# ameli/gaussian-process-param-estimation

Measured on NVIDIA B200. Metric: loglik+grad evals/s (Matern nu=2.5 dense n=20k, FP64), higher is better.
Workload: dtype f64

## Files before the change

gaussian-process-param-estimation_b200/csrc/gp_gemm.cu:

```cuda
#include "gp_common.cuh"
#include "gp_internal.h"
#include <cuda.h>
#include <algorithm>
#include <mutex>
#include <set>
#include <utility>
#include <vector>

namespace gp {

std::atomic<unsigned long long> g_launch_count{0};

struct GemmProfile {
    bool on = false;
    std::vector<cudaEvent_t> pool;
    size_t used = 0;
    double flops = 0.0;
    long long launches = 0;
    cudaEvent_t ref = nullptr;
};
static GemmProfile g_prof;
static std::mutex g_prof_mutex;

static std::mutex g_cfg_mutex;
static std::set<std::pair<int, const void*>> g_cfg_done;

int configure_once(const void* func, int smem_bytes) {
    int dev = 0;
    GP_CUDA_CHECK(cudaGetDevice(&dev));
    std::lock_guard<std::mutex> lock(g_cfg_mutex);
    std::pair<int, const void*> key(dev, func);
    if (g_cfg_done.count(key)) return 0;
    GP_CUDA_CHECK(cudaFuncSetAttribute(func, cudaFuncAttributeMaxDynamicSharedMemorySize, smem_bytes));
    g_cfg_done.insert(key);
    return 0;
}

static cudaEvent_t profile_begin(double flops, cudaStream_t stream) {
    if (!g_prof.on) return nullptr;
    std::lock_guard<std::mutex> lock(g_prof_mutex);
    while (g_prof.pool.size() < g_prof.used + 2) {
        cudaEvent_t e;
        if (cudaEventCreate(&e) != cudaSuccess) return nullptr;
        g_prof.pool.push_back(e);
    }
    cudaEvent_t e0 = g_prof.pool[g_prof.used++];
    cudaEvent_t e1 = g_prof.pool[g_prof.used++];
    g_prof.flops += flops;
    g_prof.launches++;
    cudaEventRecord(e0, stream);
    return e1;
}

static double tile_flops(int tiles_m, int tiles_n, int bn, int K, int krange, int tmask) {
    double kt = 0.0;
    for (int tm = 0; tm < tiles_m; ++tm) {
        int lim = ((tm + 1) * 128) / bn;
        int ncols = (tmask == TM_LOWER) ? (lim < tiles_n ? lim : tiles_n) : tiles_n;
        if (krange == KR_FULL) kt += (double)ncols * K;
        else if (krange == KR_A_LOWER) kt += (double)ncols * ((tm + 1) * 128 < K ? (tm + 1) * 128 : K);
        else for (int tn = 0; tn < ncols; ++tn) {
            int kb = (krange == KR_B_LOWER) ? tn * bn : (tm * 128 > tn * bn ? tm * 128 : tn * bn);
            kt += (double)(K - (kb < K ? kb : K));
        }
    }
    return 2.0 * 128.0 * bn * kt;
}

constexpr int BM = 128, WM = 64, WN = 32, MI = WM / 8, NI = WN / 8;
constexpr int RASTER_GROUP = 8;

template <int BN_>
struct TCfg {
    static constexpr int BN = BN_;
    static constexpr int BK = 16;
    static constexpr int STAGES = (BN_ == 128) ? 6 : 4;
    static constexpr int WARPS_N = BN_ / WN;
    static constexpr int CONSUMER_WARPS = (BM / WM) * WARPS_N;
    static constexpr int THREADS = (CONSUMER_WARPS + 1) * 32;
    static constexpr int A_BYTES = BM * BK * 8, B_BYTES = BN_ * BK * 8, STAGE_BYTES = A_BYTES + B_BYTES;
    static constexpr int SMEM = STAGES * STAGE_BYTES + 2048;
    static constexpr int MIN_CTAS = (BN_ == 128) ? 1 : 2;
};

__device__ __forceinline__ void mbar_init(uint32_t bar, int count) {
    asm volatile("mbarrier.init.shared::cta.b64 [%0], %1;\n" ::"r"(bar), "r"(count));
}
__device__ __forceinline__ void mbar_expect_tx(uint32_t bar, uint32_t bytes) {
    asm volatile("mbarrier.arrive.expect_tx.shared::cta.b64 _, [%0], %1;\n" ::"r"(bar), "r"(bytes) : "memory");
}
__device__ __forceinline__ void mbar_arrive(uint32_t bar) {
    asm volatile("mbarrier.arrive.shared::cta.b64 _, [%0];\n" ::"r"(bar) : "memory");
}
__device__ __forceinline__ void mbar_arrive_after(uint32_t bar, uint32_t value) {
    asm volatile(
        "{\n"
        ".reg .pred q;\n"
        "setp.ne.u32 q, %1, 0x7ff7a5c3;\n"
        "@q mbarrier.arrive.shared::cta.b64 _, [%0];\n"
        "@!q mbarrier.arrive.shared::cta.b64 _, [%0];\n"
        "}\n" ::"r"(bar), "r"(value) : "memory");
}
__device__ __forceinline__ void mbar_wait(uint32_t bar, uint32_t parity) {
    uint32_t done;
    do {
        asm volatile(
            "{\n"
            ".reg .pred p;\n"
            "mbarrier.try_wait.parity.shared::cta.b64 p, [%1], %2;\n"
            "selp.u32 %0, 1, 0, p;\n"
            "}\n" : "=r"(done) : "r"(bar), "r"(parity) : "memory");
    } while (!done);
}
__device__ __forceinline__ void tma_load_2d(uint32_t dst, const CUtensorMap* map, uint32_t bar, int c0, int c1) {
    asm volatile(
        "cp.async.bulk.tensor.2d.shared::cluster.global.mbarrier::complete_tx::bytes [%0], [%1, {%3, %4}], [%2];\n"
        ::"r"(dst), "l"(reinterpret_cast<uint64_t>(map)), "r"(bar), "r"(c0), "r"(c1) : "memory");
}
__device__ __forceinline__ void tma_load_5d(uint32_t dst, const CUtensorMap* map, uint32_t bar, int c0, int c1, int c2,
                                            int c3, int c4) {
    asm volatile(
        "cp.async.bulk.tensor.5d.shared::cluster.global.mbarrier::complete_tx::bytes [%0], [%1, {%3, %4, %5, %6, %7}], [%2];\n"
        ::"r"(dst), "l"(reinterpret_cast<uint64_t>(map)), "r"(bar), "r"(c0), "r"(c1), "r"(c2), "r"(c3), "r"(c4) : "memory");
}

template <int T>
__device__ __forceinline__ uint32_t frag_off(int mn, int kk, int t) {
    if (T == 0) {
        int chunk = (kk | ((t >> 1) << 2)) ^ (mn & 7);
        return (uint32_t)(mn * 128 + (chunk << 4) + ((t & 1) << 3));
    }
    int r = (kk & 1) | ((t & 1) << 1) | ((t >> 1) << 2) | ((kk >> 1) << 3);
    int ml = mn & 15;
    int chunk = (ml >> 1) ^ (r & 7);
    return (uint32_t)((mn >> 4) * 2048 + r * 128 + (chunk << 4) + ((ml & 1) << 3));
}

__device__ __forceinline__ double lds_f64(uint32_t addr) {
    double v;
    asm volatile("ld.shared.f64 %0, [%1];\n" : "=d"(v) : "r"(addr));
    return v;
}

template <int AT, int BT, int BN_>
__global__ void __launch_bounds__(TCfg<BN_>::THREADS, TCfg<BN_>::MIN_CTAS)
dgemm_tma_kernel(const __grid_constant__ CUtensorMap mapA, const __grid_constant__ CUtensorMap mapB, double* C, int64_t ldc,
                 int tiles_m, int tiles_n, int K, double alpha, double beta, int krange, int tmask,
                 const int* __restrict__ kbeg_tab, const int* __restrict__ kend_tab) {
    using G = TCfg<BN_>;
    constexpr int BN = G::BN, BK = G::BK, STAGES = G::STAGES;
    extern __shared__ __align__(16) unsigned char smem_raw[];

    int bid = blockIdx.x;
    int group_sz = RASTER_GROUP * tiles_n;
    int grp = bid / group_sz;
    int first_m = grp * RASTER_GROUP;
    int rows_in_grp = min(RASTER_GROUP, tiles_m - first_m);
    int rem = bid - grp * group_sz;
    int tm = first_m + rem % rows_in_grp;
    int tn = rem / rows_in_grp;
    const int m0 = tm * BM, n0 = tn * BN;
    if (tmask == TM_LOWER && n0 >= m0 + BM) return;

    int kbeg = 0, kend = K;
    if (krange == KR_A_LOWER) kend = min(K, m0 + BM);
    else if (krange == KR_B_LOWER) kbeg = min(n0, K);
    else if (krange == KR_TN_LOWER) kbeg = min(max(m0, n0), K);
    if (kbeg_tab) kbeg = max(kbeg, min(kbeg_tab[tm], K));
    if (kend_tab) kend = min(kend, kend_tab[tm]);
    kbeg = (kbeg / BK) * BK;
    const int KT = max(0, (kend - kbeg) / BK);

    const uint32_t base = ((uint32_t)__cvta_generic_to_shared(smem_raw) + 1023u) & ~1023u;
    const uint32_t bars = base + STAGES * G::STAGE_BYTES;
    const int tid = threadIdx.x, lane = tid & 31, warp = tid >> 5;

    if (tid == 0) {
#pragma unroll
        for (int s = 0; s < STAGES; ++s) {
            mbar_init(bars + 8 * s, 1);
            mbar_init(bars + 8 * (STAGES + s), G::CONSUMER_WARPS);
        }
        asm volatile("fence.mbarrier_init.release.cluster;\n" ::: "memory");
    }
    __syncthreads();

    if (warp == G::CONSUMER_WARPS) {
        if (lane == 0) {
            asm volatile("prefetch.tensormap [%0];\n" ::"l"(reinterpret_cast<uint64_t>(&mapA)) : "memory");
            asm volatile("prefetch.tensormap [%0];\n" ::"l"(reinterpret_cast<uint64_t>(&mapB)) : "memory");
            for (int kt = 0; kt < KT; ++kt) {
                const int s = kt % STAGES;
                if (kt >= STAGES) mbar_wait(bars + 8 * (STAGES + s), ((kt / STAGES) - 1) & 1);
                const uint32_t full = bars + 8 * s;
                const uint32_t sa = base + s * G::STAGE_BYTES, sb = sa + G::A_BYTES;
                const int k0 = kbeg + kt * BK;
                mbar_expect_tx(full, G::STAGE_BYTES);
                if (AT == 0) {
                    tma_load_2d(sa, &mapA, full, k0, m0);
                } else {
#pragma unroll
                    for (int j = 0; j < BM / 16; ++j) tma_load_5d(sa + j * 2048, &mapA, full, m0 + 16 * j, 0, 0, k0 >> 3, 0);
                }
                if (BT == 0) {
                    tma_load_2d(sb, &mapB, full, k0, n0);
                } else {
#pragma unroll
                    for (int j = 0; j < BN / 16; ++j) tma_load_5d(sb + j * 2048, &mapB, full, n0 + 16 * j, 0, 0, k0 >> 3, 0);
                }
            }
        }
        return;
    }

    const int g = lane >> 2, t = lane & 3;
    const int wm = (warp / G::WARPS_N) * WM, wn = (warp % G::WARPS_N) * WN;

    double acc[MI][NI][2];
#pragma unroll
    for (int i = 0; i < MI; ++i)
#pragma unroll
        for (int j = 0; j < NI; ++j) acc[i][j][0] = acc[i][j][1] = 0.0;

    if (beta != 0.0) {
        constexpr int LINES = BM * BN / 16;
        constexpr int CT = G::CONSUMER_WARPS * 32;
#pragma unroll
        for (int i = 0; i < LINES / CT; ++i) {
            int line = tid + i * CT;
            const double* pc = C + (int64_t)(m0 + line / (BN / 16)) * ldc + n0 + ((line % (BN / 16)) << 4);
            asm volatile("prefetch.global.L2 [%0];" ::"l"(pc));
        }
    }

    uint32_t aoff[4], boff[4];
#pragma unroll
    for (int kk = 0; kk < 4; ++kk) {
        aoff[kk] = frag_off<AT>(wm + g, kk, t);
        boff[kk] = frag_off<BT>(wn + g, kk, t);
    }
    for (int kt = 0; kt < KT; ++kt) {
        const int s = kt % STAGES;
        mbar_wait(bars + 8 * s, (kt / STAGES) & 1);
        const uint32_t sa = base + s * G::STAGE_BYTES, sb = sa + G::A_BYTES;
        uint32_t dep = 0;
#pragma unroll
        for (int kk = 0; kk < 4; ++kk) {
            double a[MI], b[NI];
#pragma unroll
            for (int i = 0; i < MI; ++i) {
                uint32_t o = (AT == 0) ? aoff[kk] + i * 1024 : ((aoff[kk] ^ ((i & 1) << 6)) + (i >> 1) * 2048);
                a[i] = lds_f64(sa + o);
            }
#pragma unroll
            for (int j = 0; j < NI; ++j) {
                uint32_t o = (BT == 0) ? boff[kk] + j * 1024 : ((boff[kk] ^ ((j & 1) << 6)) + (j >> 1) * 2048);
                b[j] = lds_f64(sb + o);
            }
#pragma unroll
            for (int i = 0; i < MI; ++i) dep ^= (uint32_t)__double2hiint(a[i]);
#pragma unroll
            for (int j = 0; j < NI; ++j) dep ^= (uint32_t)__double2hiint(b[j]);
#pragma unroll
            for (int i = 0; i < MI; ++i)
#pragma unroll
                for (int j = 0; j < NI; ++j) dmma884(acc[i][j][0], acc[i][j][1], a[i], b[j]);
        }
        dep = __reduce_xor_sync(0xffffffffu, dep);
        if (lane == 0) mbar_arrive_after(bars + 8 * (STAGES + s), dep);
    }

    const bool diag = (tmask == TM_LOWER) && (n0 + BN - 1 > m0);
    if (beta != 0.0 && !diag) {
#pragma unroll
        for (int i = 0; i < MI; i += 2) {
            double2 o[2][NI];
#pragma unroll
            for (int ii = 0; ii < 2; ++ii)
#pragma unroll
                for (int j = 0; j < NI; ++j)
                    o[ii][j] = *reinterpret_cast<const double2*>(C + (int64_t)(m0 + wm + (i + ii) * 8 + g) * ldc + n0 + wn + j * 8 + 2 * t);
#pragma unroll
            for (int ii = 0; ii < 2; ++ii)
#pragma unroll
                for (int j = 0; j < NI; ++j) {
                    double2 v;
                    v.x = alpha * acc[i + ii][j][0] + beta * o[ii][j].x;
                    v.y = alpha * acc[i + ii][j][1] + beta * o[ii][j].y;
                    *reinterpret_cast<double2*>(C + (int64_t)(m0 + wm + (i + ii) * 8 + g) * ldc + n0 + wn + j * 8 + 2 * t) = v;
                }
        }
        return;
    }
#pragma unroll
    for (int i = 0; i < MI; ++i) {
        const int grow = m0 + wm + i * 8 + g;
        double* crow = C + (int64_t)grow * ldc;
#pragma unroll
        for (int j = 0; j < NI; ++j) {
            const int gcol = n0 + wn + j * 8 + 2 * t;
            if (diag && gcol > grow) continue;
            double2 v;
            v.x = alpha * acc[i][j][0];
            v.y = alpha * acc[i][j][1];
            double2* p = reinterpret_cast<double2*>(crow + gcol);
            if (beta != 0.0) {
                double2 o = *p;
                v.x += beta * o.x;
                v.y += beta * o.y;
            }
            if (diag && gcol + 1 > grow) {
                crow[gcol] = v.x;
            } else {
                *p = v;
            }
        }
    }
}

typedef CUresult (*EncodeTiledFn)(CUtensorMap*, CUtensorMapDataType, cuuint32_t, void*, const cuuint64_t*, const cuuint64_t*,
                                  const cuuint32_t*, const cuuint32_t*, CUtensorMapInterleave, CUtensorMapSwizzle,
                                  CUtensorMapL2promotion, CUtensorMapFloatOOBfill);
static EncodeTiledFn g_encode = nullptr;
static int g_encode_state = 0;

static int encode_init() {
    if (g_encode_state) return g_encode_state;
    void* fn = nullptr;
    cudaDriverEntryPointQueryResult q;
    if (cudaGetDriverEntryPoint("cuTensorMapEncodeTiled", &fn, cudaEnableDefault, &q) != cudaSuccess || !fn ||
        q != cudaDriverEntryPointSuccess) {
        (void)cudaGetLastError();
        g_encode_state = -1;
        return -1;
    }
    g_encode = (EncodeTiledFn)fn;
    g_encode_state = 1;
    return 1;
}

static int make_map(CUtensorMap* map, int T, const double* P, int64_t ld, int mn, int K, int rows_per_box) {
    cuuint32_t es[5] = {1, 1, 1, 1, 1};
    CUresult r;
    if (T == 0) {
        cuuint64_t dims[2] = {(cuuint64_t)K, (cuuint64_t)mn};
        cuuint64_t strides[1] = {(cuuint64_t)ld * 8};
        cuuint32_t box[2] = {16, (cuuint32_t)rows_per_box};
        r = g_encode(map, CU_TENSOR_MAP_DATA_TYPE_FLOAT64, 2, (void*)P, dims, strides, box, es, CU_TENSOR_MAP_INTERLEAVE_NONE,
                     CU_TENSOR_MAP_SWIZZLE_128B, CU_TENSOR_MAP_L2_PROMOTION_L2_128B, CU_TENSOR_MAP_FLOAT_OOB_FILL_NONE);
    } else {
        cuuint64_t dims[5] = {(cuuint64_t)mn, 2, 2, (cuuint64_t)(K / 8), 2};
        cuuint64_t strides[4] = {(cuuint64_t)ld * 16, (cuuint64_t)ld * 8, (cuuint64_t)ld * 64, (cuuint64_t)ld * 32};
        cuuint32_t box[5] = {16, 2, 2, 2, 2};
        r = g_encode(map, CU_TENSOR_MAP_DATA_TYPE_FLOAT64, 5, (void*)P, dims, strides, box, es, CU_TENSOR_MAP_INTERLEAVE_NONE,
                     CU_TENSOR_MAP_SWIZZLE_128B, CU_TENSOR_MAP_L2_PROMOTION_L2_128B, CU_TENSOR_MAP_FLOAT_OOB_FILL_NONE);
    }
    return r == CUDA_SUCCESS ? 0 : -(int)r - 2000;
}

template <int AT, int BT, int BN_>
static int launch_tma_inst(double* C, int64_t ldc, const double* A, int64_t lda, const double* B, int64_t ldb,
                           int M, int N, int K, double alpha, double beta, int krange, int tmask, cudaStream_t stream,
                           const int* kbeg_tab, const int* kend_tab) {
    using G = TCfg<BN_>;
    if (K % G::BK) return -1;
    int tiles_m = M / BM, tiles_n = N / BN_;
    if (tiles_m == 0 || tiles_n == 0) return 0;
    int rc = configure_once((const void*)dgemm_tma_kernel<AT, BT, BN_>, G::SMEM);
    if (rc) return rc;
    const int Kmap = K > 0 ? K : 32;
    CUtensorMap mapA, mapB;
    if ((rc = make_map(&mapA, AT, A, lda, M, Kmap, BM))) return rc;
    if ((rc = make_map(&mapB, BT, B, ldb, N, Kmap, BN_))) return rc;
    cudaEvent_t e1 = profile_begin(tile_flops(tiles_m, tiles_n, BN_, K, krange, tmask), stream);
    dgemm_tma_kernel<AT, BT, BN_><<<tiles_m * tiles_n, G::THREADS, G::SMEM, stream>>>(
        mapA, mapB, C, ldc, tiles_m, tiles_n, K, alpha, beta, krange, tmask, kbeg_tab, kend_tab);
    if (e1) cudaEventRecord(e1, stream);
    GP_COUNT(1);
    GP_LAUNCH_CHECK();
    return 0;
}

static int launch_tma_bn64(int at, int bt, double* C, int64_t ldc, const double* A, int64_t lda, const double* B, int64_t ldb,
                           int M, int N, int K, double alpha, double beta, int krange, int tmask, cudaStream_t stream,
                           const int* kbeg_tab, const int* kend_tab) {
    if (at == 0 && bt == 0) return launch_tma_inst<0, 0, 64>(C, ldc, A, lda, B, ldb, M, N, K, alpha, beta, krange, tmask, stream, kbeg_tab, kend_tab);
    if (at == 0 && bt == 1) return launch_tma_inst<0, 1, 64>(C, ldc, A, lda, B, ldb, M, N, K, alpha, beta, krange, tmask, stream, kbeg_tab, kend_tab);
    if (at == 1 && bt == 1) return launch_tma_inst<1, 1, 64>(C, ldc, A, lda, B, ldb, M, N, K, alpha, beta, krange, tmask, stream, kbeg_tab, kend_tab);
    if (at == 1 && bt == 0) return launch_tma_inst<1, 0, 64>(C, ldc, A, lda, B, ldb, M, N, K, alpha, beta, krange, tmask, stream, kbeg_tab, kend_tab);
    return -4;
}

static int check_args(int at, int bt, const double* C, int64_t ldc, const double* A, int64_t lda, const double* B,
                      int64_t ldb, int M, int N, int K, bool ktab) {
    if (M < 0 || N < 0 || K < 0 || (M % BM) || (N % 128) || (K % 32)) return -1;
    if ((lda & 1) || (ldb & 1) || (ldc & 1)) return -2;
    if (((uintptr_t)A | (uintptr_t)B | (uintptr_t)C) & 15) return -3;
    const bool in_place = !ktab && C == A && C != B && ldc == lda && at == 0 && bt == 0 && N == 128;
    if ((C == A || C == B) && !in_place) return -6;
    if (encode_init() != 1) return -7;
    return in_place ? 128 : 64;
}

int launch_dgemm(int at, int bt, double* C, int64_t ldc, const double* A, int64_t lda, const double* B, int64_t ldb,
                 int M, int N, int K, double alpha, double beta, int krange, int tmask, cudaStream_t stream) {
    const int bn = check_args(at, bt, C, ldc, A, lda, B, ldb, M, N, K, false);
    if (bn < 0) return bn;
    if (bn == 128)
        return launch_tma_inst<0, 0, 128>(C, ldc, A, lda, B, ldb, M, N, K, alpha, beta, krange, tmask, stream, nullptr, nullptr);
    return launch_tma_bn64(at, bt, C, ldc, A, lda, B, ldb, M, N, K, alpha, beta, krange, tmask, stream, nullptr, nullptr);
}

int launch_dgemm_ktab(int at, int bt, double* C, int64_t ldc, const double* A, int64_t lda, const double* B, int64_t ldb,
                      int M, int N, int K, double alpha, double beta, const int* kbeg_tab, const int* kend_tab,
                      cudaStream_t stream) {
    const int bn = check_args(at, bt, C, ldc, A, lda, B, ldb, M, N, K, true);
    if (bn < 0) return bn;
    return launch_tma_bn64(at, bt, C, ldc, A, lda, B, ldb, M, N, K, alpha, beta, KR_FULL, TM_ALL, stream, kbeg_tab, kend_tab);
}


int profile_enable(int on) {
    g_prof.on = on != 0;
    g_prof.used = 0;
    g_prof.flops = 0.0;
    g_prof.launches = 0;
    if (g_prof.on) {
        if (!g_prof.ref) GP_CUDA_CHECK(cudaEventCreate(&g_prof.ref));
        GP_CUDA_CHECK(cudaDeviceSynchronize());
        GP_CUDA_CHECK(cudaEventRecord(g_prof.ref, 0));
        GP_CUDA_CHECK(cudaDeviceSynchronize());
    }
    return 0;
}

int profile_read(double* ms_sum, double* ms_union, double* flops, long long* launches) {
    GP_CUDA_CHECK(cudaDeviceSynchronize());
    std::vector<std::pair<float, float>> iv;
    double total = 0.0;
    for (size_t i = 0; i + 1 < g_prof.used; i += 2) {
        float t0 = 0.f, t1 = 0.f;
        GP_CUDA_CHECK(cudaEventElapsedTime(&t0, g_prof.ref, g_prof.pool[i]));
        GP_CUDA_CHECK(cudaEventElapsedTime(&t1, g_prof.ref, g_prof.pool[i + 1]));
        total += (double)t1 - (double)t0;
        iv.push_back(std::make_pair(t0, t1));
    }
    std::sort(iv.begin(), iv.end());
    double uni = 0.0;
    float cur0 = 0.f, cur1 = -1.f;
    for (size_t i = 0; i < iv.size(); ++i) {
        if (cur1 < cur0 || iv[i].first > cur1) {
            if (cur1 >= cur0) uni += (double)cur1 - (double)cur0;
            cur0 = iv[i].first;
            cur1 = iv[i].second;
        } else if (iv[i].second > cur1) {
            cur1 = iv[i].second;
        }
    }
    if (cur1 >= cur0) uni += (double)cur1 - (double)cur0;
    *ms_sum = total;
    *ms_union = uni;
    *flops = g_prof.flops;
    *launches = g_prof.launches;
    return 0;
}

}
```

gaussian-process-param-estimation_b200/csrc/gp_loglik.cu:

```cuda
#include "../../include/gpgp.h"
#include "gp_common.cuh"
#include "gp_internal.h"
#include "gp_matern.cuh"

namespace gp {

constexpr int MAXP = 16;
constexpr int LMAXD = 8;

__global__ void __launch_bounds__(256)
gram_partial_kernel(const double* __restrict__ A, const double* __restrict__ B, int nrows, int p, int64_t ld,
                    double* partial) {
    __shared__ double sa[64 * MAXP], sb[64 * MAXP];
    const int tid = threadIdx.x;
    const int a = tid / p, b = tid - a * p;
    double acc = 0.0;
    int rows_per_cta = (nrows + gridDim.x - 1) / gridDim.x;
    int r0 = blockIdx.x * rows_per_cta, r1 = min(nrows, r0 + rows_per_cta);
    for (int base = r0; base < r1; base += 64) {
        int cnt = min(64, r1 - base);
        __syncthreads();
        for (int idx = tid; idx < cnt * p; idx += 256) {
            int r = idx / p, c = idx - r * p;
            sa[idx] = A[(int64_t)(base + r) * ld + c];
            sb[idx] = B[(int64_t)(base + r) * ld + c];
        }
        __syncthreads();
        if (tid < p * p)
            for (int r = 0; r < cnt; ++r) acc += sa[r * p + a] * sb[r * p + b];
    }
    if (tid < p * p) partial[(int64_t)blockIdx.x * p * p + tid] = acc;
}

__global__ void sum_partials_kernel(const double* partial, int nparts, int width, double* out) {
    int t = blockIdx.x * blockDim.x + threadIdx.x;
    if (t >= width) return;
    double s = 0.0;
    for (int i = 0; i < nparts; ++i) s += partial[(int64_t)i * width + t];
    out[t] = s;
}

template <int MODE, bool WITH_DK>
__global__ void __launch_bounds__(256)
trace_tiles_kernel(const double* __restrict__ Ainv, int n, int npad, const double* __restrict__ pts, int d,
                   MaternParams mp, double* partial) {
    __shared__ double pr[LMAXD][128], pc[LMAXD][128];
    __shared__ double red[32];
    int b = blockIdx.x;
    int tm = (int)((sqrt(8.0 * b + 1.0) - 1.0) * 0.5);
    while ((tm + 1) * (tm + 2) / 2 <= b) ++tm;
    while (tm * (tm + 1) / 2 > b) --tm;
    int tn = b - tm * (tm + 1) / 2;
    const int m0 = tm * 128, n0 = tn * 128, tid = threadIdx.x;
    if (WITH_DK) {
        for (int idx = tid; idx < 128 * d; idx += 256) {
            int r = idx / d, k = idx - r * d;
            pr[k][r] = (m0 + r < n) ? pts[(int64_t)(m0 + r) * d + k] : 0.0;
            pc[k][r] = (n0 + r < n) ? pts[(int64_t)(n0 + r) * d + k] : 0.0;
        }
        __syncthreads();
    }
    double t1 = 0.0, t2 = 0.0, t3 = 0.0;
    const int tx = tid & 63, ty = tid >> 6;
    for (int r = ty; r < 128; r += 4) {
        int gi = m0 + r;
        if (gi >= n) break;
        double2 v = *reinterpret_cast<const double2*>(Ainv + (int64_t)gi * npad + n0 + 2 * tx);
        double vals[2] = {v.x, v.y};
#pragma unroll
        for (int e = 0; e < 2; ++e) {
            int gj = n0 + 2 * tx + e;
            if (gj > gi || gj >= n) continue;
            double a = vals[e];
            if (gj == gi) {
                t1 += a;
                t2 += a * a;
            } else {
                t2 += 2.0 * a * a;
                if (WITH_DK) {
                    double s = 0.0, ud = 0.0;
#pragma unroll
                    for (int k = 0; k < LMAXD; ++k)
                        if (k < d) {
                            double t = (pr[k][r] - pc[k][2 * tx + e]) * mp.inv_scale[k];
                            s += t * t;
                            if (k == mp.ddim) ud = t * t;
                        }
                    double val, dval;
                    matern_value_drho<MODE>(sqrt(s), mp, &val, &dval);
                    if (mp.ddim >= 0) dval = (s > 0.0) ? dval * (ud / s) * mp.inv_scale[mp.ddim] : 0.0;
                    t3 += 2.0 * a * dval;
                }
            }
        }
    }
    t1 = block_sum(t1, red);
    t2 = block_sum(t2, red);
    t3 = block_sum(t3, red);
    if (tid == 0) {
        partial[(int64_t)b * 3 + 0] = t1;
        partial[(int64_t)b * 3 + 1] = t2;
        partial[(int64_t)b * 3 + 2] = t3;
    }
}

__global__ void __launch_bounds__(256)
frob_lower_kernel(const double* __restrict__ W, int n, int npad, double* partial) {
    __shared__ double red[32];
    int tm = blockIdx.y, tn = blockIdx.x;
    double s = 0.0;
    if (tn <= tm) {
        int m0 = tm * 128, n0 = tn * 128;
        for (int idx = threadIdx.x; idx < 128 * 64; idx += 256) {
            int r = idx >> 6, c = (idx & 63) * 2;
            int gi = m0 + r;
            if (gi >= n) break;
            double2 v = *reinterpret_cast<const double2*>(W + (int64_t)gi * npad + n0 + c);
            if (n0 + c <= gi) s += v.x * v.x;
            if (n0 + c + 1 <= gi) s += v.y * v.y;
        }
    }
    s = block_sum(s, red);
    if (threadIdx.x == 0) partial[blockIdx.y * gridDim.x + blockIdx.x] = s;
}

constexpr int SSP = MAXP + 1;
constexpr int DKR = 16;
template <int MODE, int PP>
__global__ void __launch_bounds__(256)
dk_apply_kernel(const double* __restrict__ pts, int n, int d, MaternParams mp, const double* __restrict__ S, int p,
                int64_t lds, double* __restrict__ V) {
    constexpr int SP = PP + 1;
    __shared__ double pcs[LMAXD][128];
    __shared__ double ss[128 * SP];
    const int tid = threadIdx.x, lane = tid & 31, warp = tid >> 5;
    const int g0 = blockIdx.x * DKR + warp * 2;
    double pi[2][LMAXD];
#pragma unroll
    for (int r = 0; r < 2; ++r)
#pragma unroll
        for (int k = 0; k < LMAXD; ++k) pi[r][k] = (k < d && g0 + r < n) ? pts[(int64_t)(g0 + r) * d + k] : 0.0;
    double acc[2][PP];
#pragma unroll
    for (int r = 0; r < 2; ++r)
#pragma unroll
        for (int c = 0; c < PP; ++c) acc[r][c] = 0.0;
    for (int j0 = 0; j0 < n; j0 += 128) {
        __syncthreads();
        for (int idx = tid; idx < 128 * d; idx += 256) {
            int r = idx / d, k = idx - r * d;
            pcs[k][r] = (j0 + r < n) ? pts[(int64_t)(j0 + r) * d + k] : 0.0;
        }
        for (int idx = tid; idx < 128 * p; idx += 256) {
            int r = idx / p, c = idx - r * p;
            ss[r * SP + c] = (j0 + r < n) ? S[(int64_t)(j0 + r) * lds + c] : 0.0;
        }
        __syncthreads();
#pragma unroll
        for (int t = 0; t < 4; ++t) {
            const int jj = t * 32 + lane;
            const int gj = j0 + jj;
#pragma unroll
            for (int r = 0; r < 2; ++r) {
                const int gi = g0 + r;
                if (gi >= n || gj >= n || gj == gi) continue;
                double s2 = 0.0, ud = 0.0;
#pragma unroll
                for (int k = 0; k < LMAXD; ++k)
                    if (k < d) {
                        double u = (pi[r][k] - pcs[k][jj]) * mp.inv_scale[k];
                        s2 += u * u;
                        if (k == mp.ddim) ud = u * u;
                    }
                double val, dval;
                matern_value_drho<MODE>(sqrt(s2), mp, &val, &dval);
                if (mp.ddim >= 0) dval = (s2 > 0.0) ? dval * (ud / s2) * mp.inv_scale[mp.ddim] : 0.0;
#pragma unroll
                for (int c = 0; c < PP; ++c)
                    if (c < p) acc[r][c] += dval * ss[jj * SP + c];
            }
        }
    }
    const int rows128 = ((n + 127) / 128) * 128;
#pragma unroll
    for (int r = 0; r < 2; ++r)
#pragma unroll
        for (int c = 0; c < PP; ++c)
            if (c < p) {
                const double v = warp_sum(acc[r][c]);
                if (lane == 0 && g0 + r < rows128) V[(int64_t)(g0 + r) * lds + c] = (g0 + r < n) ? v : 0.0;
            }
}

template <int MODE>
static void launch_dk_apply(const double* pts, int n, int d, const MaternParams& mp, const double* S, int p, int64_t lds,
                            double* V, cudaStream_t s) {
    const unsigned grid = (unsigned)((((n + 127) / 128) * 128) / DKR);
    if (p <= 8) dk_apply_kernel<MODE, 8><<<grid, 256, 0, s>>>(pts, n, d, mp, S, p, lds, V);
    else dk_apply_kernel<MODE, MAXP><<<grid, 256, 0, s>>>(pts, n, d, mp, S, p, lds, V);
}

__global__ void __launch_bounds__(256)
symm_skinny_kernel(const double* __restrict__ K, int n, int npad, const double* __restrict__ X, int p, double* __restrict__ Y) {
    __shared__ double xs[128 * SSP];
    const int tid = threadIdx.x, lane = tid & 31, warp = tid >> 5;
    const int r0 = blockIdx.x * 32 + warp * 4;
    double acc[4][MAXP];
#pragma unroll
    for (int r = 0; r < 4; ++r)
#pragma unroll
        for (int c = 0; c < MAXP; ++c) acc[r][c] = 0.0;
    for (int j0 = 0; j0 < npad; j0 += 128) {
        __syncthreads();
        for (int idx = tid; idx < 128 * p; idx += 256) {
            int r = idx / p, c = idx - r * p;
            xs[r * SSP + c] = (j0 + r < n) ? X[(int64_t)(j0 + r) * p + c] : 0.0;
        }
        __syncthreads();
#pragma unroll
        for (int q = 0; q < 4; ++q) {
            int j = lane + 32 * q;
            double kv[4];
#pragma unroll
            for (int r = 0; r < 4; ++r) kv[r] = K[(int64_t)(r0 + r) * npad + j0 + j];
#pragma unroll
            for (int c = 0; c < MAXP; ++c)
                if (c < p) {
                    double x = xs[j * SSP + c];
#pragma unroll
                    for (int r = 0; r < 4; ++r) acc[r][c] += kv[r] * x;
                }
        }
    }
#pragma unroll
    for (int r = 0; r < 4; ++r)
#pragma unroll
        for (int c = 0; c < MAXP; ++c)
            if (c < p) {
                double v = warp_sum(acc[r][c]);
                if (lane == 0) Y[(int64_t)(r0 + r) * p + c] = (r0 + r < n) ? v : 0.0;
            }
}

template <int PP>
__global__ void __launch_bounds__(256)
tril_skinny_kernel(const double* __restrict__ W, int npad, const double* __restrict__ X, int p, double* __restrict__ Y) {
    constexpr int SP = PP + 1;
    __shared__ double xs[128 * SP];
    const int tid = threadIdx.x, lane = tid & 31, warp = tid >> 5;
    const int rb = ((int)gridDim.x - 1 - (int)blockIdx.x) * 32, r0 = rb + warp * 4;
    double acc[4][PP];
#pragma unroll
    for (int r = 0; r < 4; ++r)
#pragma unroll
        for (int c = 0; c < PP; ++c) acc[r][c] = 0.0;
    for (int j0 = 0; j0 < rb + 32; j0 += 128) {
        __syncthreads();
        for (int idx = tid; idx < 128 * p; idx += 256) {
            int r = idx / p, c = idx - r * p;
            xs[r * SP + c] = X[(int64_t)(j0 + r) * p + c];
        }
        __syncthreads();
#pragma unroll
        for (int q = 0; q < 4; ++q) {
            int j = lane + 32 * q;
            double kv[4];
#pragma unroll
            for (int r = 0; r < 4; ++r) kv[r] = (j0 + j <= r0 + r) ? W[(int64_t)(r0 + r) * npad + j0 + j] : 0.0;
#pragma unroll
            for (int c = 0; c < PP; ++c)
                if (c < p) {
                    double x = xs[j * SP + c];
#pragma unroll
                    for (int r = 0; r < 4; ++r) acc[r][c] += kv[r] * x;
                }
        }
    }
#pragma unroll
    for (int r = 0; r < 4; ++r)
#pragma unroll
        for (int c = 0; c < PP; ++c)
            if (c < p) {
                double v = warp_sum(acc[r][c]);
                if (lane == 0) Y[(int64_t)(r0 + r) * p + c] = v;
            }
}

constexpr int TCH = 1024;
template <int PP>
__global__ void __launch_bounds__(256)
trilT_skinny_partial_kernel(const double* __restrict__ W, int npad, const double* __restrict__ X, int p, double* __restrict__ partial) {
    constexpr int SP = PP + 1;
    __shared__ double xs[128 * SP];
    __shared__ double comb[128 * SP];
    const int tid = threadIdx.x;
    const int i0 = blockIdx.x * 128, kc = blockIdx.y;
    const int il = tid & 127, half = tid >> 7, i = i0 + il;
    int kbeg = kc * TCH, kend = min(npad, kbeg + TCH);
    double acc[PP];
#pragma unroll
    for (int c = 0; c < PP; ++c) acc[c] = 0.0;
    if (kend > i0) {
        if (kbeg < i0) kbeg = i0;
        for (int k0 = kbeg; k0 < kend; k0 += 128) {
            __syncthreads();
            for (int idx = tid; idx < 128 * p; idx += 256) {
                int r = idx / p, c = idx - r * p;
                xs[r * SP + c] = X[(int64_t)(k0 + r) * p + c];
            }
            __syncthreads();
#pragma unroll 4
            for (int kk = half; kk < 128; kk += 2) {
                int k = k0 + kk;
                double w = (k >= i) ? W[(int64_t)k * npad + i] : 0.0;
#pragma unroll
                for (int c = 0; c < PP; ++c)
                    if (c < p) acc[c] += w * xs[kk * SP + c];
            }
        }
    }
    __syncthreads();
    if (half == 1)
#pragma unroll
        for (int c = 0; c < PP; ++c) comb[il * SP + c] = acc[c];
    __syncthreads();
    if (half == 0)
        for (int c = 0; c < p; ++c) partial[((int64_t)kc * npad + i) * p + c] = acc[c] + comb[il * SP + c];
}

__global__ void trilT_reduce_kernel(const double* __restrict__ partial, int npad, int p, int nchunks, double* __restrict__ Y) {
    int64_t t = (int64_t)blockIdx.x * blockDim.x + threadIdx.x;
    if (t >= (int64_t)npad * p) return;
    int i = (int)(t / p);
    double s = 0.0;
    for (int kc = i / TCH; kc < nchunks; ++kc) s += partial[(int64_t)kc * npad * p + t];
    Y[t] = s;
}

__global__ void __launch_bounds__(256)
finalize_out_kernel(double* out, const double* logdet, const double* tr_parts, int ntiles, const double* frob_parts,
                    int nfrob, const int* info, int flags) {
    __shared__ double red[32];
    double t1 = 0.0, t2 = 0.0, t3 = 0.0;
    if (flags & 2) {
        for (int i = threadIdx.x; i < ntiles; i += 256) {
            t1 += tr_parts[3 * i];
            t2 += tr_parts[3 * i + 1];
            t3 += tr_parts[3 * i + 2];
        }
    } else if (flags & 1) {
        for (int i = threadIdx.x; i < nfrob; i += 256) t1 += frob_parts[i];
    }
    t1 = block_sum(t1, red);
    t2 = block_sum(t2, red);
    t3 = block_sum(t3, red);
    if (threadIdx.x == 0) {
        out[0] = *logdet;
        out[1] = t1;
        out[2] = t2;
        out[3] = t3;
        out[4] = (double)(*info);
        out[5] = out[6] = out[7] = 0.0;
    }
}

static size_t align256(size_t x) { return (x + 255) & ~(size_t)255; }

struct LoglikWs {
    double* S;
    double* V;
    double* V2;
    double* logdet;
    double* gram;
    double* tr;
    double* frob;
    int* info;
    double* tpart;
    void* potri;
    size_t total;
};

static LoglikWs carve(void* ws, int64_t npad, int p) {
    LoglikWs w;
    char* base = (char*)ws;
    size_t off = 0;
    int64_t T = npad / 128;
    auto take = [&](size_t bytes) { size_t o = off; off += align256(bytes); return base ? base + o : (char*)nullptr; };
    w.S = (double*)take(sizeof(double) * npad * MAXP);
    w.V = (double*)take(sizeof(double) * npad * MAXP);
    w.V2 = (double*)take(sizeof(double) * npad * MAXP);
    w.logdet = (double*)take(sizeof(double) * 4);
    w.gram = (double*)take(sizeof(double) * 296 * MAXP * MAXP);
    w.tr = (double*)take(sizeof(double) * (T * (T + 1) / 2) * 3);
    w.frob = (double*)take(sizeof(double) * T * T);
    w.info = (int*)take(sizeof(int) * 4);
    w.tpart = (double*)take(sizeof(double) * (npad / TCH + 1) * npad * MAXP);
    w.potri = (void*)take((size_t)gp_potri_workspace_bytes(npad));
    w.total = off;
    (void)p;
    return w;
}

static int gram(const double* A, const double* B, int nrows, int p, int64_t ld, double* partial, double* out, cudaStream_t s) {
    int parts = 296;
    gram_partial_kernel<<<parts, 256, 0, s>>>(A, B, nrows, p, ld, partial);
    sum_partials_kernel<<<(p * p + 127) / 128, 128, 0, s>>>(partial, parts, p * p, out);
    GP_COUNT(2);
    GP_LAUNCH_CHECK();
    return 0;
}

static int solve_with_inverse(const double* W, int npad, double* S, double* tmp, int p, double* tpart, cudaStream_t s) {
    int nchunks = (npad + TCH - 1) / TCH;
    if (p <= 8) {
        tril_skinny_kernel<8><<<npad / 32, 256, 0, s>>>(W, npad, S, p, tmp);
        trilT_skinny_partial_kernel<8><<<dim3(npad / 128, nchunks), 256, 0, s>>>(W, npad, tmp, p, tpart);
    } else {
        tril_skinny_kernel<MAXP><<<npad / 32, 256, 0, s>>>(W, npad, S, p, tmp);
        trilT_skinny_partial_kernel<MAXP><<<dim3(npad / 128, nchunks), 256, 0, s>>>(W, npad, tmp, p, tpart);
    }
    trilT_reduce_kernel<<<(unsigned)(((int64_t)npad * p + 255) / 256), 256, 0, s>>>(tpart, npad, p, nchunks, S);
    GP_COUNT(3);
    GP_LAUNCH_CHECK();
    return 0;
}

template <int MODE>
static int grad_reductions(const double* Ainv, int n, int npad, const double* pts, int d, const MaternParams& mp, bool with_dk,
                           const LoglikWs& w, int p, double* outQ, cudaStream_t s) {
    int T = npad / 128, tiles = T * (T + 1) / 2;
    if (with_dk) {
        trace_tiles_kernel<MODE, true><<<tiles, 256, 0, s>>>(Ainv, n, npad, pts, d, mp, w.tr);
        launch_dk_apply<MODE>(pts, n, d, mp, w.S, p, p, w.V, s);
        GP_COUNT(2);
        GP_LAUNCH_CHECK();
        return gram(w.S, w.V, n, p, p, w.gram, outQ, s);
    }
    trace_tiles_kernel<MODE, false><<<tiles, 256, 0, s>>>(Ainv, n, npad, pts, d, mp, w.tr);
    GP_COUNT(1);
    GP_LAUNCH_CHECK();
    return 0;
}

}

using namespace gp;

extern "C" {

int gp_symm_skinny(const double* K, int64_t n, int64_t npad, const double* X, int64_t p, double* Y, void* stream) {
    if (!K || !X || !Y || n <= 0 || npad != gp_padded_size(n) || p <= 0 || p > MAXP) return -1;
    symm_skinny_kernel<<<(unsigned)(npad / 32), 256, 0, (cudaStream_t)stream>>>(K, (int)n, (int)npad, X, (int)p, Y);
    GP_COUNT(1);
    GP_LAUNCH_CHECK();
    return 0;
}

int gp_dk_apply(const double* points, int64_t n, int64_t d, const double* scale_host, double nu, const double* S, int64_t p,
                int64_t lds, double* V, void* stream) {
    if (!points || !scale_host || !S || !V || n <= 0 || d <= 0 || d > LMAXD || p <= 0 || p > MAXP || lds < p) return -1;
    MaternParams mp;
    mp.nu = nu; mp.coef = 0.0; mp.sq2nu = 0.0;
    for (int k = 0; k < d; ++k) {
        if (!(scale_host[k] > 0.0) || scale_host[k] != scale_host[0]) return -4;
        mp.inv_scale[k] = 1.0 / scale_host[k];
    }
    mp.inv_rho = 1.0 / scale_host[0];
    int mode = matern_mode_of(nu);
    if (mode == MAT_GENERAL) {
        mp.coef = pow(2.0, 1.0 - nu) / tgamma(nu);
        mp.sq2nu = sqrt(2.0 * nu);
    }
    cudaStream_t s = (cudaStream_t)stream;
    switch (mode) {
        case MAT_05: launch_dk_apply<MAT_05>(points, (int)n, (int)d, mp, S, (int)p, lds, V, s); break;
        case MAT_15: launch_dk_apply<MAT_15>(points, (int)n, (int)d, mp, S, (int)p, lds, V, s); break;
        case MAT_25: launch_dk_apply<MAT_25>(points, (int)n, (int)d, mp, S, (int)p, lds, V, s); break;
        case MAT_GAUSS: launch_dk_apply<MAT_GAUSS>(points, (int)n, (int)d, mp, S, (int)p, lds, V, s); break;
        default: launch_dk_apply<MAT_GENERAL>(points, (int)n, (int)d, mp, S, (int)p, lds, V, s); break;
    }
    GP_COUNT(1);
    GP_LAUNCH_CHECK();
    return 0;
}

int64_t gp_traces_workspace_bytes(int64_t npad) {
    int64_t T = npad / 128;
    return (int64_t)sizeof(double) * (T * (T + 1) / 2 * 3 + T * T + 64);
}

int gp_inverse_traces(const double* M, int64_t n, int64_t npad, int kind, double* out_dev, void* ws, void* stream) {
    if (!M || !out_dev || !ws || n <= 0 || npad != gp_padded_size(n) || (kind != 0 && kind != 1)) return -1;
    cudaStream_t s = (cudaStream_t)stream;
    int T = (int)(npad / 128), tiles = T * (T + 1) / 2;
    double* tr = (double*)ws;
    double* frob = tr + (int64_t)tiles * 3;
    double* misc = frob + (int64_t)T * T;
    GP_CUDA_CHECK(cudaMemsetAsync(misc, 0, sizeof(double) * 8, s));
    MaternParams mp;
    mp.nu = 0; mp.coef = 0; mp.sq2nu = 0; mp.inv_rho = 0;
    if (kind == 0) frob_lower_kernel<<<dim3(T, T), 256, 0, s>>>(M, (int)n, (int)npad, frob);
    else trace_tiles_kernel<MAT_05, false><<<tiles, 256, 0, s>>>(M, (int)n, (int)npad, nullptr, 0, mp, tr);
    finalize_out_kernel<<<1, 256, 0, s>>>(out_dev, misc, tr, tiles, frob, T * T, (const int*)(misc + 2), kind == 0 ? 1 : 2);
    GP_COUNT(2);
    GP_LAUNCH_CHECK();
    return 0;
}

__global__ void sum_trace3_kernel(const double* __restrict__ tr, int tiles, double* out) {
    __shared__ double red[32];
    double s = 0.0;
    for (int i = threadIdx.x; i < tiles; i += blockDim.x) s += tr[(int64_t)i * 3 + 2];
    s = block_sum(s, red);
    if (threadIdx.x == 0) out[0] = s;
}

int gp_loglik_dense_dscale(const double* Ainv, int64_t n, int64_t npad, int64_t p, const double* points, int64_t d,
                           const double* scale_host, double nu, int64_t dim, void* ws, double* out_dim, void* stream) {
    if (!Ainv || !points || !scale_host || !ws || !out_dim || n <= 0 || npad != gp_padded_size(n) || p <= 0 || p > MAXP ||
        d <= 0 || d > LMAXD || dim < 0 || dim >= d)
        return -1;
    cudaStream_t s = (cudaStream_t)stream;
    LoglikWs w = carve(ws, npad, (int)p);
    MaternParams mp;
    mp.nu = nu; mp.coef = 0.0; mp.sq2nu = 0.0; mp.inv_rho = 1.0; mp.ddim = (int)dim;
    for (int k = 0; k < d; ++k) {
        if (!(scale_host[k] > 0.0)) return -4;
        mp.inv_scale[k] = 1.0 / scale_host[k];
    }
    int mode = matern_mode_of(nu);
    if (mode == MAT_GENERAL) {
        mp.coef = pow(2.0, 1.0 - nu) / tgamma(nu);
        mp.sq2nu = sqrt(2.0 * nu);
    }
    const int N = (int)n, NP = (int)npad, P = (int)p;
    int rc;
    switch (mode) {
        case MAT_05: rc = grad_reductions<MAT_05>(Ainv, N, NP, points, (int)d, mp, true, w, P, out_dim + 1, s); break;
        case MAT_15: rc = grad_reductions<MAT_15>(Ainv, N, NP, points, (int)d, mp, true, w, P, out_dim + 1, s); break;
        case MAT_25: rc = grad_reductions<MAT_25>(Ainv, N, NP, points, (int)d, mp, true, w, P, out_dim + 1, s); break;
        case MAT_GAUSS: rc = grad_reductions<MAT_GAUSS>(Ainv, N, NP, points, (int)d, mp, true, w, P, out_dim + 1, s); break;
        default: rc = grad_reductions<MAT_GENERAL>(Ainv, N, NP, points, (int)d, mp, true, w, P, out_dim + 1, s); break;
    }
    if (rc) return rc;
    int T = NP / 128;
    sum_trace3_kernel<<<1, 256, 0, s>>>(w.tr, T * (T + 1) / 2, out_dim);
    GP_COUNT(1);
    GP_LAUNCH_CHECK();
    return 0;
}

int64_t gp_loglik_workspace_bytes(int64_t npad) { return (int64_t)carve(nullptr, npad, MAXP).total; }

int64_t gp_loglik_out_len(int64_t p) { return 8 + 4 * p * p; }

int gp_loglik_dense(const double* K, int64_t n, int64_t npad, const double* R, int64_t p, double eta, int flags,
                    const double* points, int64_t d, const double* scale_host, double nu, double* A, double* W,
                    void* potrf_ws, void* ws, double* out, void* stream) {
    if (!K || !R || !A || !potrf_ws || !ws || !out || n <= 0 || npad != gp_padded_size(n) || p <= 0 || p > MAXP) return -1;
    if ((flags & 3) && !W) return -2;
    if ((flags & 4) && (!(flags & 2) || !points || !scale_host || d <= 0 || d > LMAXD)) return -3;
    if ((flags & 8) && !(flags & 3)) return -5;
    cudaStream_t s = (cudaStream_t)stream;
    LoglikWs w = carve(ws, npad, (int)p);
    const int N = (int)n, NP = (int)npad, P = (int)p;
    int rc;
    if ((rc = gp_shift_copy(K, n, npad, eta, A, stream))) return rc;
    if ((rc = gp_potrf_f64(A, n, npad, w.info, potrf_ws, stream))) return rc;
    if ((rc = gp_logdet_from_chol(A, n, npad, w.logdet, stream))) return rc;
    GP_CUDA_CHECK(cudaMemcpyAsync(w.S, R, sizeof(double) * npad * p, cudaMemcpyDeviceToDevice, s));
    int T = NP / 128;
    if (flags & 3) {
        if ((rc = gp_trtri_f64(A, W, npad, potrf_ws, w.potri, stream))) return rc;
        if ((rc = solve_with_inverse(W, NP, w.S, w.V, P, w.tpart, s))) return rc;
    } else {
        if ((rc = gp_potrs_f64(A, npad, potrf_ws, w.S, p, p, stream))) return rc;
    }
    double* G = out + 8;
    double* H = G + p * p;
    double* Q = H + p * p;
    if ((rc = gram(R, w.S, N, P, p, w.gram, G, s))) return rc;
    if ((rc = gram(w.S, w.S, N, P, p, w.gram, H, s))) return rc;
    double* T3 = Q + p * p;
    GP_CUDA_CHECK(cudaMemsetAsync(Q, 0, sizeof(double) * 2 * p * p, s));
    if (flags & 8) {
        GP_CUDA_CHECK(cudaMemcpyAsync(w.V2, w.S, sizeof(double) * npad * p, cudaMemcpyDeviceToDevice, s));
        if ((rc = solve_with_inverse(W, NP, w.V2, w.V, P, w.tpart, s))) return rc;
        if ((rc = gram(w.S, w.V2, N, P, p, w.gram, T3, s))) return rc;
    }
    if (flags & 2) {
        if ((rc = gp_lauum_f64(W, A, npad, stream))) return rc;
        bool with_dk = (flags & 4) != 0;
        MaternParams mp;
        mp.nu = nu; mp.coef = 0.0; mp.sq2nu = 0.0; mp.inv_rho = 0.0;
        int mode = MAT_05;
        if (with_dk) {
            for (int k = 0; k < d; ++k) {
                if (!(scale_host[k] > 0.0) || scale_host[k] != scale_host[0]) return -4;
                mp.inv_scale[k] = 1.0 / scale_host[k];
            }
            mp.inv_rho = 1.0 / scale_host[0];
            mode = matern_mode_of(nu);
            if (mode == MAT_GENERAL) {
                mp.coef = pow(2.0, 1.0 - nu) / tgamma(nu);
                mp.sq2nu = sqrt(2.0 * nu);
            }
        }
        switch (mode) {
            case MAT_05: rc = grad_reductions<MAT_05>(A, N, NP, points, (int)d, mp, with_dk, w, P, Q, s); break;
            case MAT_15: rc = grad_reductions<MAT_15>(A, N, NP, points, (int)d, mp, with_dk, w, P, Q, s); break;
            case MAT_25: rc = grad_reductions<MAT_25>(A, N, NP, points, (int)d, mp, with_dk, w, P, Q, s); break;
            case MAT_GAUSS: rc = grad_reductions<MAT_GAUSS>(A, N, NP, points, (int)d, mp, with_dk, w, P, Q, s); break;
            default: rc = grad_reductions<MAT_GENERAL>(A, N, NP, points, (int)d, mp, with_dk, w, P, Q, s); break;
        }
        if (rc) return rc;
    } else if (flags & 1) {
        frob_lower_kernel<<<dim3(T, T), 256, 0, s>>>(W, N, NP, w.frob);
        GP_COUNT(1);
        GP_LAUNCH_CHECK();
    }
    finalize_out_kernel<<<1, 256, 0, s>>>(out, w.logdet, w.tr, T * (T + 1) / 2, w.frob, T * T, w.info, flags);
    GP_COUNT(1);
    GP_LAUNCH_CHECK();
    return 0;
}

}
```

Before: 4.056.

## Fuse dK apply into trace tile kernel and launch only lower-triangular GEMM tiles

The trace kernel now also builds the dK tile in shared memory and multiplies it against S for both the row and column blocks. Per-tile partial products go to a workspace aliased on the potri buffer, and a small kernel reduces them into V. This replaces the separate launch_dk_apply pass, which recomputed the Matern derivative. Separately, the TMA DGEMM launches only lower-triangular tiles, using a grouped raster mapping found by binary search, so CTAs no longer launch just to exit. The cost is more shared memory and partial-buffer traffic, plus reuse of the potri workspace.

```diff
diff --git a/gaussian-process-param-estimation_b200/csrc/gp_gemm.cu b/gaussian-process-param-estimation_b200/csrc/gp_gemm.cu
--- a/gaussian-process-param-estimation_b200/csrc/gp_gemm.cu
+++ b/gaussian-process-param-estimation_b200/csrc/gp_gemm.cu
@@ -142,6 +142,48 @@
     return v;
 }
 
+__host__ __device__ __forceinline__ int lower_cols(int tm, int tiles_n, int bn) {
+    return min(tiles_n, (tm + 1) * (BM / bn));
+}
+__host__ __device__ __forceinline__ long long lower_tiles_before(int t, int tiles_n, int bn) {
+    const long long r = BM / bn, t0 = min((long long)t, tiles_n / r);
+    return r * t0 * (t0 + 1) / 2 + ((long long)t - t0) * tiles_n;
+}
+
+__device__ __forceinline__ void tile_of_block(int bid, int tiles_m, int tiles_n, int bn, int tmask, int& tm, int& tn) {
+    if (tmask != TM_LOWER) {
+        const int group_sz = RASTER_GROUP * tiles_n;
+        const int grp = bid / group_sz;
+        const int first_m = grp * RASTER_GROUP;
+        const int rows_in_grp = min(RASTER_GROUP, tiles_m - first_m);
+        const int rem = bid - grp * group_sz;
+        tm = first_m + rem % rows_in_grp;
+        tn = rem / rows_in_grp;
+        return;
+    }
+    int lo = 0, hi = (tiles_m - 1) / RASTER_GROUP;
+    while (lo < hi) {
+        const int mid = (lo + hi + 1) >> 1;
+        if (lower_tiles_before(mid * RASTER_GROUP, tiles_n, bn) <= bid) lo = mid;
+        else hi = mid - 1;
+    }
+    const int first_m = lo * RASTER_GROUP;
+    const int rows_in_grp = min(RASTER_GROUP, tiles_m - first_m);
+    int rem = bid - (int)lower_tiles_before(first_m, tiles_n, bn);
+    int col = 0;
+    for (int i = 0; i < rows_in_grp; ++i) {
+        const int ci = lower_cols(first_m + i, tiles_n, bn), h = rows_in_grp - i, cnt = (ci - col) * h;
+        if (rem < cnt) {
+            tm = first_m + i + rem % h;
+            tn = col + rem / h;
+            return;
+        }
+        rem -= cnt;
+        col = ci;
+    }
+    tm = tn = 0;
+}
+
 template <int AT, int BT, int BN_>
 __global__ void __launch_bounds__(TCfg<BN_>::THREADS, TCfg<BN_>::MIN_CTAS)
 dgemm_tma_kernel(const __grid_constant__ CUtensorMap mapA, const __grid_constant__ CUtensorMap mapB, double* C, int64_t ldc,
@@ -151,16 +193,9 @@
     constexpr int BN = G::BN, BK = G::BK, STAGES = G::STAGES;
     extern __shared__ __align__(16) unsigned char smem_raw[];
 
-    int bid = blockIdx.x;
-    int group_sz = RASTER_GROUP * tiles_n;
-    int grp = bid / group_sz;
-    int first_m = grp * RASTER_GROUP;
-    int rows_in_grp = min(RASTER_GROUP, tiles_m - first_m);
-    int rem = bid - grp * group_sz;
-    int tm = first_m + rem % rows_in_grp;
-    int tn = rem / rows_in_grp;
+    int tm, tn;
+    tile_of_block(blockIdx.x, tiles_m, tiles_n, BN, tmask, tm, tn);
     const int m0 = tm * BM, n0 = tn * BN;
-    if (tmask == TM_LOWER && n0 >= m0 + BM) return;
 
     int kbeg = 0, kend = K;
     if (krange == KR_A_LOWER) kend = min(K, m0 + BM);
@@ -372,8 +407,9 @@
     CUtensorMap mapA, mapB;
     if ((rc = make_map(&mapA, AT, A, lda, M, Kmap, BM))) return rc;
     if ((rc = make_map(&mapB, BT, B, ldb, N, Kmap, BN_))) return rc;
+    const long long blocks = (tmask == TM_LOWER) ? lower_tiles_before(tiles_m, tiles_n, BN_) : (long long)tiles_m * tiles_n;
     cudaEvent_t e1 = profile_begin(tile_flops(tiles_m, tiles_n, BN_, K, krange, tmask), stream);
-    dgemm_tma_kernel<AT, BT, BN_><<<tiles_m * tiles_n, G::THREADS, G::SMEM, stream>>>(
+    dgemm_tma_kernel<AT, BT, BN_><<<(unsigned)blocks, G::THREADS, G::SMEM, stream>>>(
         mapA, mapB, C, ldc, tiles_m, tiles_n, K, alpha, beta, krange, tmask, kbeg_tab, kend_tab);
     if (e1) cudaEventRecord(e1, stream);
     GP_COUNT(1);
diff --git a/gaussian-process-param-estimation_b200/csrc/gp_loglik.cu b/gaussian-process-param-estimation_b200/csrc/gp_loglik.cu
--- a/gaussian-process-param-estimation_b200/csrc/gp_loglik.cu
+++ b/gaussian-process-param-estimation_b200/csrc/gp_loglik.cu
@@ -2,6 +2,7 @@
 #include "gp_common.cuh"
 #include "gp_internal.h"
 #include "gp_matern.cuh"
+#include <algorithm>
 
 namespace gp {
 
@@ -40,27 +41,21 @@
     out[t] = s;
 }
 
-template <int MODE, bool WITH_DK>
-__global__ void __launch_bounds__(256)
-trace_tiles_kernel(const double* __restrict__ Ainv, int n, int npad, const double* __restrict__ pts, int d,
-                   MaternParams mp, double* partial) {
-    __shared__ double pr[LMAXD][128], pc[LMAXD][128];
-    __shared__ double red[32];
-    int b = blockIdx.x;
-    int tm = (int)((sqrt(8.0 * b + 1.0) - 1.0) * 0.5);
+__device__ __forceinline__ void lower_tile(int b, int& tm, int& tn) {
+    tm = (int)((sqrt(8.0 * b + 1.0) - 1.0) * 0.5);
     while ((tm + 1) * (tm + 2) / 2 <= b) ++tm;
     while (tm * (tm + 1) / 2 > b) --tm;
-    int tn = b - tm * (tm + 1) / 2;
+    tn = b - tm * (tm + 1) / 2;
+}
+
+__global__ void __launch_bounds__(256)
+trace_tiles_kernel(const double* __restrict__ Ainv, int n, int npad, double* partial) {
+    __shared__ double red[32];
+    const int b = blockIdx.x;
+    int tm, tn;
+    lower_tile(b, tm, tn);
     const int m0 = tm * 128, n0 = tn * 128, tid = threadIdx.x;
-    if (WITH_DK) {
-        for (int idx = tid; idx < 128 * d; idx += 256) {
-            int r = idx / d, k = idx - r * d;
-            pr[k][r] = (m0 + r < n) ? pts[(int64_t)(m0 + r) * d + k] : 0.0;
-            pc[k][r] = (n0 + r < n) ? pts[(int64_t)(n0 + r) * d + k] : 0.0;
-        }
-        __syncthreads();
-    }
-    double t1 = 0.0, t2 = 0.0, t3 = 0.0;
+    double t1 = 0.0, t2 = 0.0;
     const int tx = tid & 63, ty = tid >> 6;
     for (int r = ty; r < 128; r += 4) {
         int gi = m0 + r;
@@ -77,23 +72,116 @@
                 t2 += a * a;
             } else {
                 t2 += 2.0 * a * a;
-                if (WITH_DK) {
-                    double s = 0.0, ud = 0.0;
-#pragma unroll
-                    for (int k = 0; k < LMAXD; ++k)
-                        if (k < d) {
-                            double t = (pr[k][r] - pc[k][2 * tx + e]) * mp.inv_scale[k];
-                            s += t * t;
-                            if (k == mp.ddim) ud = t * t;
-                        }
-                    double val, dval;
-                    matern_value_drho<MODE>(sqrt(s), mp, &val, &dval);
-                    if (mp.ddim >= 0) dval = (s > 0.0) ? dval * (ud / s) * mp.inv_scale[mp.ddim] : 0.0;
-                    t3 += 2.0 * a * dval;
+            }
+        }
+    }
+    t1 = block_sum(t1, red);
+    t2 = block_sum(t2, red);
+    if (tid == 0) {
+        partial[(int64_t)b * 3 + 0] = t1;
+        partial[(int64_t)b * 3 + 1] = t2;
+        partial[(int64_t)b * 3 + 2] = 0.0;
+    }
+}
+
+constexpr int DKC = 32;
+constexpr int DKP = 129;
+template <int PP>
+static int trace_dk_smem(int d) { return (int)sizeof(double) * (2 * d * 128 + 2 * 128 * (PP + 1) + DKC * DKP); }
+
+template <int MODE, int PP>
+__global__ void __launch_bounds__(256)
+trace_dk_tiles_kernel(const double* __restrict__ Ainv, int n, int npad, const double* __restrict__ pts, int d,
+                      MaternParams mp, const double* __restrict__ S, int p, double* __restrict__ partial,
+                      double* __restrict__ dkpart) {
+    constexpr int SP = PP + 1, HC = PP / 2;
+    extern __shared__ double smem[];
+    double* pr = smem;
+    double* pc = pr + d * 128;
+    double* sr = pc + d * 128;
+    double* sc = sr + 128 * SP;
+    double* D = sc + 128 * SP;
+    __shared__ double red[32];
+    const int b = blockIdx.x, T = npad / 128;
+    int tm, tn;
+    lower_tile(b, tm, tn);
+    const int m0 = tm * 128, n0 = tn * 128, tid = threadIdx.x;
+    for (int idx = tid; idx < 128 * d; idx += 256) {
+        int r = idx / d, k = idx - r * d;
+        pr[k * 128 + r] = (m0 + r < n) ? pts[(int64_t)(m0 + r) * d + k] : 0.0;
+        pc[k * 128 + r] = (n0 + r < n) ? pts[(int64_t)(n0 + r) * d + k] : 0.0;
+    }
+    for (int idx = tid; idx < 128 * p; idx += 256) {
+        int r = idx / p, c = idx - r * p;
+        sr[r * SP + c] = (m0 + r < n) ? S[(int64_t)(m0 + r) * p + c] : 0.0;
+        sc[r * SP + c] = (n0 + r < n) ? S[(int64_t)(n0 + r) * p + c] : 0.0;
+    }
+    double t1 = 0.0, t2 = 0.0, t3 = 0.0;
+    const int tx = tid & 63, ty = tid >> 6;
+    const int cj = tid & 127, c0 = (tid >> 7) * HC;
+    double cacc[HC];
+#pragma unroll
+    for (int c = 0; c < HC; ++c) cacc[c] = 0.0;
+    double* rowpart = dkpart + ((int64_t)tm * T + tn) * 128 * p;
+    for (int r0 = 0; r0 < 128; r0 += DKC) {
+        __syncthreads();
+        for (int r = r0 + ty; r < r0 + DKC; r += 4) {
+            const int gi = m0 + r;
+            double vals[2] = {0.0, 0.0};
+            if (gi < n) {
+                double2 v = *reinterpret_cast<const double2*>(Ainv + (int64_t)gi * npad + n0 + 2 * tx);
+                vals[0] = v.x;
+                vals[1] = v.y;
+            }
+#pragma unroll
+            for (int e = 0; e < 2; ++e) {
+                const int gj = n0 + 2 * tx + e;
+                double dv = 0.0;
+                if (gi < n && gj <= gi && gj < n) {
+                    const double a = vals[e];
+                    if (gj == gi) {
+                        t1 += a;
+                        t2 += a * a;
+                    } else {
+                        t2 += 2.0 * a * a;
+                        double s = 0.0, ud = 0.0;
+#pragma unroll
+                        for (int k = 0; k < LMAXD; ++k)
+                            if (k < d) {
+                                double t = (pr[k * 128 + r] - pc[k * 128 + 2 * tx + e]) * mp.inv_scale[k];
+                                s += t * t;
+                                if (k == mp.ddim) ud = t * t;
+                            }
+                        double val, dval;
+                        matern_value_drho<MODE>(sqrt(s), mp, &val, &dval);
+                        if (mp.ddim >= 0) dval = (s > 0.0) ? dval * (ud / s) * mp.inv_scale[mp.ddim] : 0.0;
+                        t3 += 2.0 * a * dval;
+                        dv = dval;
+                    }
                 }
-            }
-        }
-    }
+                D[(r - r0) * DKP + 2 * tx + e] = dv;
+            }
+        }
+        __syncthreads();
+        for (int o = tid; o < DKC * p; o += 256) {
+            const int r = o / p, c = o - r * p;
+            double acc = 0.0;
+#pragma unroll 8
+            for (int j = 0; j < 128; ++j) acc += D[r * DKP + j] * sc[j * SP + c];
+            rowpart[(int64_t)(r0 + r) * p + c] = acc;
+        }
+#pragma unroll 4
+        for (int r = 0; r < DKC; ++r) {
+            const double dv = D[r * DKP + cj];
+#pragma unroll
+            for (int c = 0; c < HC; ++c) cacc[c] += dv * sr[(r0 + r) * SP + c0 + c];
+        }
+    }
+    __syncthreads();
+    double* colpart = dkpart + ((int64_t)tn * T + tm) * 128 * p + (int64_t)cj * p;
+#pragma unroll
+    for (int c = 0; c < HC; ++c)
+        if (c0 + c < p) colpart[c0 + c] = (tm == tn) ? colpart[c0 + c] + cacc[c] : cacc[c];
     t1 = block_sum(t1, red);
     t2 = block_sum(t2, red);
     t3 = block_sum(t3, red);
@@ -102,6 +190,16 @@
         partial[(int64_t)b * 3 + 1] = t2;
         partial[(int64_t)b * 3 + 2] = t3;
     }
+}
+
+__global__ void dk_partial_reduce_kernel(const double* __restrict__ dkpart, int n, int npad, int p, double* __restrict__ V) {
+    const int64_t t = (int64_t)blockIdx.x * blockDim.x + threadIdx.x;
+    if (t >= (int64_t)npad * p) return;
+    const int i = (int)(t / p), c = (int)(t - (int64_t)i * p), T = npad / 128;
+    const double* src = dkpart + ((int64_t)(i >> 7) * T * 128 + (i & 127)) * p + c;
+    double s = 0.0;
+    for (int u = 0; u < T; ++u) s += src[(int64_t)u * 128 * p];
+    V[t] = (i < n) ? s : 0.0;
 }
 
 __global__ void __launch_bounds__(256)
@@ -377,6 +475,7 @@
     int* info;
     double* tpart;
     void* potri;
+    double* dkpart;
     size_t total;
 };
 
@@ -395,7 +494,9 @@
     w.frob = (double*)take(sizeof(double) * T * T);
     w.info = (int*)take(sizeof(int) * 4);
     w.tpart = (double*)take(sizeof(double) * (npad / TCH + 1) * npad * MAXP);
-    w.potri = (void*)take((size_t)gp_potri_workspace_bytes(npad));
+    const size_t dk_bytes = sizeof(double) * T * T * 128 * MAXP;
+    w.potri = (void*)take(std::max((size_t)gp_potri_workspace_bytes(npad), dk_bytes));
+    w.dkpart = (double*)w.potri;
     w.total = off;
     (void)p;
     return w;
@@ -425,18 +526,30 @@
     return 0;
 }
 
+template <int MODE, int PP>
+static int launch_trace_dk(const double* Ainv, int n, int npad, const double* pts, int d, const MaternParams& mp,
+                           const LoglikWs& w, int p, cudaStream_t s) {
+    if (int rc = configure_once((const void*)trace_dk_tiles_kernel<MODE, PP>, trace_dk_smem<PP>(LMAXD))) return rc;
+    const int T = npad / 128, tiles = T * (T + 1) / 2;
+    trace_dk_tiles_kernel<MODE, PP><<<tiles, 256, trace_dk_smem<PP>(d), s>>>(Ainv, n, npad, pts, d, mp, w.S, p, w.tr,
+                                                                             w.dkpart);
+    return 0;
+}
+
 template <int MODE>
 static int grad_reductions(const double* Ainv, int n, int npad, const double* pts, int d, const MaternParams& mp, bool with_dk,
                            const LoglikWs& w, int p, double* outQ, cudaStream_t s) {
     int T = npad / 128, tiles = T * (T + 1) / 2;
     if (with_dk) {
-        trace_tiles_kernel<MODE, true><<<tiles, 256, 0, s>>>(Ainv, n, npad, pts, d, mp, w.tr);
-        launch_dk_apply<MODE>(pts, n, d, mp, w.S, p, p, w.V, s);
+        int rc = (p <= 8) ? launch_trace_dk<MODE, 8>(Ainv, n, npad, pts, d, mp, w, p, s)
+                          : launch_trace_dk<MODE, MAXP>(Ainv, n, npad, pts, d, mp, w, p, s);
+        if (rc) return rc;
+        dk_partial_reduce_kernel<<<(unsigned)(((int64_t)npad * p + 255) / 256), 256, 0, s>>>(w.dkpart, n, npad, p, w.V);
         GP_COUNT(2);
         GP_LAUNCH_CHECK();
         return gram(w.S, w.V, n, p, p, w.gram, outQ, s);
     }
-    trace_tiles_kernel<MODE, false><<<tiles, 256, 0, s>>>(Ainv, n, npad, pts, d, mp, w.tr);
+    trace_tiles_kernel<<<tiles, 256, 0, s>>>(Ainv, n, npad, w.tr);
     GP_COUNT(1);
     GP_LAUNCH_CHECK();
     return 0;
@@ -497,10 +610,8 @@
     double* frob = tr + (int64_t)tiles * 3;
     double* misc = frob + (int64_t)T * T;
     GP_CUDA_CHECK(cudaMemsetAsync(misc, 0, sizeof(double) * 8, s));
-    MaternParams mp;
-    mp.nu = 0; mp.coef = 0; mp.sq2nu = 0; mp.inv_rho = 0;
     if (kind == 0) frob_lower_kernel<<<dim3(T, T), 256, 0, s>>>(M, (int)n, (int)npad, frob);
-    else trace_tiles_kernel<MAT_05, false><<<tiles, 256, 0, s>>>(M, (int)n, (int)npad, nullptr, 0, mp, tr);
+    else trace_tiles_kernel<<<tiles, 256, 0, s>>>(M, (int)n, (int)npad, tr);
     finalize_out_kernel<<<1, 256, 0, s>>>(out_dev, misc, tr, tiles, frob, T * T, (const int*)(misc + 2), kind == 0 ? 1 : 2);
     GP_COUNT(2);
     GP_LAUNCH_CHECK();
```

After: 4.119, median of 6. +1.6%, better.
